# pepborrell/cool-chic

Hardware: AMD Instinct MI355X
Metric: decoded Mpixel/s (Synth+ARM+upsample) @1280x720, all GPUs (higher is better)
Workload: dtype f32; 1 GPU; 1280x720 YUV420 8-bit frames, hop/c3x decoder (arm 16x2, syn 48-1/3-1/3-3r/3-3r, 7 latent grids), float forward ARM+rate -> upsampling -> synthesis -> 420 post; parallelism=image-parallel x1, kernels=ARM | upsampling pyramid | fused last-upsampling+synthesis+post (one stream)

## Files before the change

cool-chic_amd/csrc/fwd_syn.hip:

```cpp
#include <stdlib.h>
#include <type_traits>

#include "fwd_common.h"

using namespace ccmi_fwd;

namespace {

constexpr int kThreads = 256;


#ifndef CCMI_FUSED_RH
#define CCMI_FUSED_RH 32
#endif
#ifndef CCMI_FUSED_THREADS
#define CCMI_FUSED_THREADS 512
#endif
constexpr int kFThreads = CCMI_FUSED_THREADS;
constexpr int kRW = 64, kRH = CCMI_FUSED_RH;
constexpr int kRowsPerThread = kRH / (kFThreads / kRW);
constexpr int kNW = kFThreads / 64;

__device__ __forceinline__ float *at(float *base, uint32_t i) { return (float *)((char *)base + i * 4u); }
__device__ __forceinline__ float ldu(const float *base, uint64_t byte) { return *(const float *)((const char *)base + byte); }
__device__ __forceinline__ uint64_t off64(uint32_t byte, uint32_t z)
{
    uint64_t o = ((uint64_t)z << 32) | byte;
    asm volatile("" : "+v"(o));
    return o;
}

__device__ __forceinline__ void store_out(const FusedArgs &A, float *out, int64_t plane, int m, int gy, int gx, float v,
                                          const float *lut8)
{
    const uint32_t pl = (uint32_t)plane, px = (uint32_t)(gy * A.W + gx);
    if (A.qmax <= 0.f) {
        *at(out, m * pl + px) = v;
        return;
    }
    const float q = lut8 ? lut8[(int)fminf(fmaxf(rintf(v * 255.f), 0.f), 255.f)]
                         : fminf(fmaxf(rintf(v * A.qmax) / A.qmax, 0.f), 1.f);
    if (!A.yuv420 || m == 0) {
        *at(out, m * pl + px) = q;
    } else if (!(gy & 1) && !(gx & 1) && (gy >> 1) < (A.H >> 1) && (gx >> 1) < (A.W >> 1)) {
        const uint32_t cp = (uint32_t)((A.H >> 1) * (A.W >> 1));
        *at(out, pl + (m - 1) * cp + (uint32_t)((gy >> 1) * (A.W >> 1) + (gx >> 1))) = q;
    }
}

typedef float v4f __attribute__((ext_vector_type(4)));
__device__ __forceinline__ v4f mfma16(float a, float b, v4f c) { return __builtin_amdgcn_mfma_f32_16x16x4f32(a, b, c, 0, 0, 0); }

__device__ __forceinline__ void rows_transpose4(const float (&v)[4], float (&t)[4])
{
    const auto p = __builtin_amdgcn_permlane16_swap(__float_as_uint(v[0]), __float_as_uint(v[1]), false, false);
    const auto q = __builtin_amdgcn_permlane16_swap(__float_as_uint(v[2]), __float_as_uint(v[3]), false, false);
    const auto a = __builtin_amdgcn_permlane32_swap(p[0], q[0], false, false);
    const auto b = __builtin_amdgcn_permlane32_swap(p[1], q[1], false, false);
    t[0] = __uint_as_float(a[0]);
    t[1] = __uint_as_float(b[0]);
    t[2] = __uint_as_float(a[1]);
    t[3] = __uint_as_float(b[1]);
}

typedef const __attribute__((address_space(4))) char *kernarg_ptr;
__device__ __forceinline__ kernarg_ptr fresh_kernargs()
{
    kernarg_ptr p = (kernarg_ptr)__builtin_amdgcn_kernarg_segment_ptr();
    asm volatile("" : "+s"(p));
    return p;
}

#if defined(CCMI_ARM_STAMPS)
__device__ unsigned long long g_fstamp[8];
#define FSTAMP(k)                                                                  \
    do {                                                                           \
        __syncthreads();                                                           \
        const unsigned long long _t = __builtin_amdgcn_s_memtime();                \
        if (threadIdx.x == 0) atomicAdd(&g_fstamp[k], _t - t_prev);                \
        t_prev = _t;                                                               \
    } while (0)
#else
#define FSTAMP(k)
#endif

using FT = UpsTile<8, 7, kRH, kRW>;
constexpr int kHsRows = kRH / 2 + 1 + FT::NS - 1;
constexpr int kHrRows = kRH + 7 - 1;
constexpr int kSW = kRW / 2 + 1 + FT::NS - 1 + 3;
constexpr int kTW = kRW + 7 - 1 + 2;

constexpr int fused_groups(int cin, bool ups) { return ups && cin - 1 >= 4 ? 2 : 1; }
constexpr int fused_carry_floats(int cmid) { return kMaxSp * 2 * cmid * kRW; }
constexpr int fused_lds_floats(int cin, int cmid, bool ups)
{
    const int C = ups ? cin - 1 : 0, GC = (C + fused_groups(cin, ups) - 1) / fused_groups(cin, ups);
    const int raw = ups ? GC * kHsRows * kSW + kHrRows * kTW : 0;
    const int stage = ups ? GC * kHsRows * kRW + kHrRows * kRW : 0;
    const int xr = 2 * cmid * kFThreads;
    const int b0 = xr > raw ? xr : raw;
    int b1 = xr > stage ? xr : stage;
    b1 = b1 > kMaxHid * 16 + 256 ? b1 : kMaxHid * 16 + 256;
    return b0 + b1 + fused_carry_floats(cmid) + 256;
}
constexpr int fused_wpe(int cin, int cmid, bool ups, bool mh = false)
{
#ifdef CCMI_FUSED_WPE
    if (!mh) return CCMI_FUSED_WPE;
#endif
    return !mh && 4 * fused_lds_floats(cin, cmid, ups) <= 160 * 1024 / 3 ? 6 : 4;
}

template <int CIN, int CMID, bool UPS, bool MH = false, int HID = 0, bool FOLD = false>
__global__ __launch_bounds__(kFThreads) __attribute__((amdgpu_waves_per_eu(fused_wpe(CIN, CMID, UPS, MH)))) void syn_fused_kernel(FusedArgs Ak, LevelArgs Uk, LevelArgs U2k)
{
    static_assert(!FOLD || (UPS && CIN >= 3), "the fold needs the fused level-1 -> 0 step and a level-2 stack");
    constexpr int NR = kRowsPerThread;
    constexpr int C = UPS ? CIN - 1 : 0, NG = fused_groups(CIN, UPS), GC = (C + NG - 1) / NG;
    constexpr int kRaw = UPS ? GC * kHsRows * kSW + kHrRows * kTW : 0;
    constexpr int kBuf0 = 2 * CMID * kFThreads > kRaw ? 2 * CMID * kFThreads : kRaw;
    constexpr int kTot = fused_lds_floats(CIN, CMID, UPS);
    __shared__ __attribute__((aligned(16))) float s_pool[kTot];
    float *s_st = s_pool;
    float *s_yt = s_st + GC * kHsRows * kSW;
    float *s_hs = s_pool + kBuf0;
    float *s_hr = s_hs + GC * kHsRows * kRW;
    float *s_lut8 = s_pool + kTot - 256;
    float *s_carry = s_lut8 - fused_carry_floats(CMID);
#if defined(CCMI_ARM_STAMPS)
    unsigned long long t_prev = __builtin_amdgcn_s_memtime();
#endif
    float(*s_head)[16] = reinterpret_cast<float(*)[16]>(s_pool + kBuf0);
    float *s_w1p = s_pool + kBuf0 + kMaxHid * 16;
    static_assert(CIN + 1 + CMID <= 16, "hidden-unit record");
    constexpr int kRecVecs = (CIN + 1 + CMID + 3) / 4;

    const int wt = xcd_order(blockIdx.x, gridDim.x);
    const int b0 = wt / Ak.ntiles, tile = wt - b0 * Ak.ntiles;
    const int ri = tile / Ak.tiles_x;
    const int nwin = Ak.run_base + (ri < Ak.run_extra ? 1 : 0);
    const int y0 = kRH * (ri * Ak.run_base + min(ri, Ak.run_extra)) - 2 * Ak.n_sp * ri;
    const int x0 = (tile - ri * Ak.tiles_x) * (kRW - 2 * Ak.n_sp);
    const int oy0 = y0 - Ak.n_sp, ox0 = x0 - Ak.n_sp;
    if (Ak.qmax == 255.f) s_lut8[threadIdx.x & 255] = (float)(threadIdx.x & 255) / 255.f;
#pragma clang loop unroll(disable)
    for (int win = 0; win < nwin; ++win) {
    auto tixf = []() __attribute__((always_inline)) {
        int t = threadIdx.x;
        asm volatile("" : "+v"(t));
        return t;
    };
    const auto kargs = fresh_kernargs();
    constexpr size_t kOffU = (sizeof(FusedArgs) + alignof(LevelArgs) - 1) / alignof(LevelArgs) * alignof(LevelArgs);
    constexpr size_t kOffU2 = (kOffU + sizeof(LevelArgs) + alignof(LevelArgs) - 1) / alignof(LevelArgs) * alignof(LevelArgs);
    const FusedArgs &A = *(const FusedArgs *)kargs;
    const LevelArgs &U = *(const LevelArgs *)(kargs + kOffU);
    const LevelArgs &U2 = *(const LevelArgs *)(kargs + kOffU2);
    const int halo = A.n_sp;
    int b = b0, ox = ox0;
    asm volatile("" : "+s"(b), "+s"(ox));
    const int oy = oy0 + kRH * win;
    const cfloat_ptr prm = (cfloat_ptr)(size_t)(A.params + (int64_t)b * A.pstride);
    const float *in = A.in + (int64_t)b * A.in_stride;
    float *out = A.out + (int64_t)b * A.out_stride;
    const int64_t plane = (int64_t)A.H * A.W;
    int c, rb, gx, cxg;
    auto reidx = [&]() {
        int t = threadIdx.x;
        asm volatile("" : "+v"(t));
        c = t & (kRW - 1);
        rb = (t >> 6) * NR;
        gx = ox + c;
        cxg = clampi(gx, A.W - 1);
    };

    const float *lut8 = A.qmax == 255.f ? s_lut8 : nullptr;
    constexpr int kHeadRegs = (kMaxHid * 16 + kFThreads - 1) / kFThreads;
    constexpr bool kScaledRelu = HID > 0 && !MH;
    constexpr float kW0Scale = kScaledRelu ? 0x1p-32f : 1.f, kW1Scale = kScaledRelu ? 0x1p32f : 1.f;
    float hv[kHeadRegs];
    auto load_head = [&]() {
        const int tid = tixf();
#pragma unroll
        for (int k = 0; k < kHeadRegs; ++k) {
            const int i = tid + k * kFThreads, j = i >> 4, f = i & 15;
            float v = 0.f;
            if (i < kMaxHid * 16 && A.n_head == 2 && j < A.hid) {
                if (f < CIN) v = prm[A.w0_off + j * CIN + f] * kW0Scale;
                else if (f == CIN) v = prm[A.b0_off + j] * kW0Scale;
                else if (f <= CIN + CMID) v = prm[A.w1_off + (f - CIN - 1) * A.hid + j] * kW1Scale;
            }
            hv[k] = v;
        }
    };
    auto stage_head = [&]() {
        const int tid = tixf();
#pragma unroll
        for (int k = 0; k < kHeadRegs; ++k) {
            const int i = tid + k * kFThreads, j = i >> 4, f = i & 15;
            if (i < kMaxHid * 16 && f <= CIN + CMID) s_head[j][f] = hv[k];
        }
        if constexpr (MH) {
            constexpr int n = (HID / 16) * 4 * CMID * 4;
            static_assert(n <= kFThreads, "one entry per thread");
            const int i = tid;
            if (i < n) {
                const int u4 = i & 3, m = (i >> 2) % CMID, lgi = (i / (4 * CMID)) & 3, mt = i / (16 * CMID);
                s_w1p[i] = prm[A.w1_off + m * A.hid + 16 * mt + 4 * lgi + u4];
            }
        }
    };
    reidx();
    if constexpr (!UPS) {
        load_head();
        stage_head();
        __syncthreads();
    }

    float x[NR][CIN];
    const int Ya = clampi(oy, A.H - 1), Xa = clampi(ox, A.W - 1);
    const bool interior = oy >= 0 && oy + kRH <= A.H;
    if constexpr (UPS) {
        float wu[8], wr[7];
        const cfloat_ptr uprm = (cfloat_ptr)(size_t)(U.params + (int64_t)b * U.pstride);
#pragma unroll
        for (int k = 0; k < 8; ++k) wu[k] = uprm[U.up_off + k];
#pragma unroll
        for (int k = 0; k < 7; ++k) wr[k] = uprm[U.pre_off + k];
        const int jbase = Ya / 2 + FT::D0, ibase = Xa / 2 + FT::D0;
        const int wv = __builtin_amdgcn_readfirstlane((int)(tixf() >> 6));
        const int lane = tixf() & 63;
        constexpr int kSR = GC * kHsRows, kSU = (kSR + kNW - 1) / kNW;
        constexpr int kLU = (kHrRows + kNW - 1) / kNW;
        static_assert(kSW <= 64 && kTW <= 128 && kTW > 64 && kHsRows >= kNW, "lane = raw column, one row wrap per step");
        const float *src = U.src + (int64_t)b * U.src_stride;
        const float *rs = U.ref_src + (int64_t)b * U.ref_stride;
        float sv[NG][kSU], tv[kLU][2];
        bool tin[2];
        {
            const int splane = U.hs * U.ws;
            const uint32_t zhi = (uint32_t)tixf() >> 31;
            const uint64_t scol = off64(4u * (uint32_t)clampi(ibase + (lane < kSW ? lane : kSW - 1), U.ws - 1), zhi);
#pragma unroll
            for (int G = 0; G < NG; ++G)
#pragma unroll
                for (int u = 0; u < kSU; ++u) {
                    if constexpr (FOLD) break;
                    const int r = wv + kNW * u;
                    const int c0 = (kNW * u) / kHsRows, tb = kHsRows * (c0 + 1) - kNW * u;
                    const int lc = c0 + (wv >= tb ? 1 : 0), jj = r - lc * kHsRows;
                    sv[G][u] = 0.f;
                    if ((u < kSU - 1 || r < kSR) && G * GC + lc < C) {
                        const int row = (G * GC + lc) * splane + clampi(jbase + jj, U.hs - 1) * U.ws;
#if defined(CCMI_DIAG_NOLOAD)
                        sv[G][u] = 0.001f * (float)(jj + scol);
#else
                        sv[G][u] = ldu(src + row, scol);
#endif
                    }
                }
            uint64_t tx[2];
#pragma unroll
            for (int h = 0; h < 2; ++h) {
                const int X = Xa - 3 + (lane + 64 * h < kTW ? lane + 64 * h : kTW - 1);
                tin[h] = X >= 0 && X < U.wd;
                tx[h] = off64(4u * (uint32_t)clampi(X, U.wd - 1), zhi);
            }
#pragma unroll
            for (int u = 0; u < kLU; ++u) {
                const int yr = wv + kNW * u;
                const int Y = Ya - 3 + yr;
                const int row = clampi(Y, U.hd - 1) * U.wd;
#pragma unroll
                for (int h = 0; h < 2; ++h) {
#if defined(CCMI_DIAG_NOLOAD)
                    tv[u][h] = 0.001f * (float)(yr + tx[h]);
#else
                    tv[u][h] = ldu(rs + row, tx[h]);
#endif
                }
            }
        }
        if constexpr (FOLD) {
            constexpr int C2 = CIN - 2;
            constexpr int kFLR = kHsRows + 6, kFLW = kSW + 6, kFLP = kFLW + 1;
            constexpr int kFP = 40;
            constexpr int kF2R = (kHsRows - 1) / 2 + 1 + FT::NS - 1;
            constexpr int kF2W = (kSW - 1) / 2 + 1 + FT::NS - 1, kF2P = kF2W + 1;
            static_assert(kFP >= kSW, "pass pitch");
            float *f_lat = s_pool;
            float *f_ref = f_lat + kFLR * kFLP;
            float *f_src = f_ref + kFLR * kFP;
            float *f_h2 = f_src + C2 * kF2R * kF2P;
            static_assert(kFLR * kFLP + kFLR * kFP + C2 * kF2R * (kF2P + kFP) <= kTot - 256 - fused_carry_floats(CMID), "fold tiles fit before the carry rows");
            const int hs1 = U.hs, ws1 = U.ws, hs2 = U2.hs, ws2 = U2.ws;
            const int R0 = clampi(jbase, hs1 - 1), R1 = clampi(jbase + kHsRows - 1, hs1 - 1);
            const int C0 = clampi(ibase, ws1 - 1);
            const int r2 = (R0 >> 1) + FT::D0, c2 = (C0 >> 1) + FT::D0;
            const cfloat_ptr uprm2 = (cfloat_ptr)(size_t)(U2.params + (int64_t)b * U2.pstride);
            float wu2[8], wr2[7];
#pragma unroll
            for (int k = 0; k < 8; ++k) wu2[k] = uprm2[U2.up_off + k];
#pragma unroll
            for (int k = 0; k < 7; ++k) wr2[k] = uprm2[U2.pre_off + k];
            const int tid = tixf();
            {
                const float *l1 = U2.ref_src + (int64_t)b * U2.ref_stride;
                const float *s2 = U2.src + (int64_t)b * U2.src_stride;
                constexpr int NL = (kFLR * kFLW + kFThreads - 1) / kFThreads;
                constexpr int NS2 = (C2 * kF2R * kF2W + kFThreads - 1) / kFThreads;
                float lv[NL], sv2[NS2];
#pragma unroll
                for (int u = 0; u < NL; ++u) {
                    const int i = tid + u * kFThreads, r = i / kFLW, c = i - r * kFLW;
                    const int Y = R0 - 3 + r, X = C0 - 3 + c;
                    lv[u] = (i < kFLR * kFLW && Y >= 0 && Y < hs1 && X >= 0 && X < ws1) ? l1[Y * ws1 + X] : 0.f;
                }
#pragma unroll
                for (int u = 0; u < NS2; ++u) {
                    const int i = tid + u * kFThreads, ch = i / (kF2R * kF2W), rem = i - ch * (kF2R * kF2W);
                    const int r = rem / kF2W, c = rem - r * kF2W;
                    sv2[u] = i < C2 * kF2R * kF2W
                                 ? s2[(ch * hs2 + clampi(r2 + r, hs2 - 1)) * ws2 + clampi(c2 + c, ws2 - 1)]
                                 : 0.f;
                }
#pragma unroll
                for (int u = 0; u < NL; ++u) {
                    const int i = tid + u * kFThreads, r = i / kFLW, c = i - r * kFLW;
                    if (i < kFLR * kFLW) f_lat[r * kFLP + c] = U2.ref_quant ? rintf(U2.gain * lv[u]) : lv[u];
                }
#pragma unroll
                for (int u = 0; u < NS2; ++u) {
                    const int i = tid + u * kFThreads, ch = i / (kF2R * kF2W), rem = i - ch * (kF2R * kF2W);
                    const int r = rem / kF2W, c = rem - r * kF2W;
                    if (i < C2 * kF2R * kF2W) f_src[(ch * kF2R + r) * kF2P + c] = U2.src_quant ? rintf(U2.gain * sv2[u]) : sv2[u];
                }
            }
            __syncthreads();
            for (int i = tid; i < kFLR * kSW; i += kFThreads) {
                const int r = i / kSW, c = i - r * kSW;
                const float *p = f_lat + r * kFLP + c;
                float acc = 0.f;
#pragma unroll
                for (int k = 0; k < 7; ++k) acc = fmaf(wr2[k], p[k], acc);
                f_ref[r * kFP + c] = acc;
            }
            {
                constexpr int NQ = kSW / 2 + 1;
                const int q0 = C0 >> 1;
                for (int i = tid; i < C2 * kF2R * NQ; i += kFThreads) {
                    const int ch = i / (kF2R * NQ), rem = i - ch * (kF2R * NQ), r = rem / NQ, q = rem - r * NQ;
                    const float *p = f_src + (ch * kF2R + r) * kF2P + q;
                    float e = 0.f, o = 0.f;
#pragma unroll
                    for (int m = 0; m < FT::NS; ++m) {
// ... 63 lines not shown
            constexpr int G = decltype(GI)::value;
            if constexpr (G > 0) __syncthreads();
#pragma unroll
            for (int u = 0; u < kSU; ++u) {
                const int r = wv + kNW * u;
                if ((u < kSU - 1 || r < kSR) && lane < kSW)
                    s_st[r * kSW + lane] = U.src_quant ? rintf(U.gain * sv[G][u]) : sv[G][u];
            }
            if constexpr (G == 0) {
#pragma unroll
                for (int u = 0; u < kLU; ++u) {
                    const int yr = wv + kNW * u;
                    if (yr >= kHrRows) continue;
                    const int Y = Ya - 3 + yr;
                    const bool yin = Y >= 0 && Y < U.hd;
#pragma unroll
                    for (int h = 0; h < 2; ++h) {
                        const float v = U.ref_quant ? rintf(U.gain * tv[u][h]) : tv[u][h];
                        if (lane + 64 * h < kTW) s_yt[yr * kTW + lane + 64 * h] = (yin && tin[h]) ? v : 0.f;
                    }
                }
            }
            __builtin_amdgcn_fence(__ATOMIC_RELEASE, "wavefront");
            __builtin_amdgcn_wave_barrier();
            __builtin_amdgcn_fence(__ATOMIC_ACQUIRE, "wavefront");
            if constexpr (G == 0) FSTAMP(0);
            {
                const int odd = Xa & 1;
                const int k = lane & 31, hsel = lane >> 5;
                const int xe = 2 * k - odd;
                static_assert(32 + FT::NS - 1 < kSW, "pair 32 reads stay inside the source row");
                auto pair = [&](int r, int kk, int xw) {
                    const float *sr = s_st + r * kSW + kk;
                    f2 eo = f2(0.f);
#pragma unroll
                    for (int m = 0; m < FT::NS; ++m) eo = __builtin_elementwise_fma(wp[m], f2(sr[m]), eo);
                    float *hrow = s_hs + r * kRW;
                    if (xw >= 0) hrow[xw] = eo.x;
                    if (xw + 1 < kRW) hrow[xw + 1] = eo.y;
                };
#pragma unroll
                for (int u = 0; u < kSU; u += 2) {
                    const int r = wv + kNW * (u + hsel);
                    if (u + 1 < kSU - 1 || r < kSR) pair(r, k, xe);
                }
                if (odd) {
                    const int r = wv + kNW * lane;
                    if (lane < kSU && r < kSR) pair(r, 32, 63);
                }
                if constexpr (G == 0) {
#pragma unroll
                    for (int u = 0; u < kLU; ++u) {
                        const int yr = wv + kNW * u;
                        if (yr >= kHrRows) continue;
                        const float *tr = s_yt + yr * kTW + lane;
                        float acc = 0.f;
#pragma unroll
                        for (int q = 0; q < 7; ++q) acc = fmaf(wr[q], tr[q], acc);
                        s_hr[yr * kRW + lane] = acc;
                    }
                }
            }
            __syncthreads();
            if constexpr (G == 0) FSTAMP(1);
            const int xi = cxg - Xa;
            if (interior) {
                auto gather = [&](auto par) {
                    constexpr int P = decltype(par)::value;
                    if constexpr (G == 0) {
                        float h[NR + 6];
#pragma unroll
                        for (int k = 0; k < NR + 6; ++k) h[k] = s_hr[(rb + k) * kRW + xi];
#pragma unroll
                        for (int p = 0; p < NR; ++p) {
                            float acc = 0.f;
#pragma unroll
                            for (int k = 0; k < 7; ++k) acc = fmaf(wr[k], h[p + k], acc);
                            x[p][0] = acc + s_yt[(rb + p + 3) * kTW + xi + 3];
                        }
                    }
                    constexpr int NH = FT::NS + (NR / 2) - 1 + P;
                    const int j0 = rb / 2;
#pragma unroll
                    for (int lc = 0; lc < GC; ++lc) {
                        constexpr int dummy = 0;
                        (void)dummy;
                        const int k = 1 + G * GC + lc;
                        if (k >= CIN) break;
                        float h[NH];
#pragma unroll
                        for (int m = 0; m < NH; ++m) h[m] = s_hs[(lc * kHsRows + j0 + m) * kRW + xi];
#pragma unroll
                        for (int p = 0; p < NR; ++p) {
                            const int a = (P + p) & 1, off = (P + p) >> 1;
                            float acc = 0.f;
#pragma unroll
                            for (int m = 0; m < FT::NS; ++m) {
                                const int te = FT::tap(0, FT::D0 + m), to = FT::tap(1, FT::D0 + m);
                                if ((a ? to : te) >= 0) acc = fmaf(wu[a ? to : te], h[off + m], acc);
                            }
                            x[p][k] = acc;
                        }
                    }
                };
                if (oy & 1) gather(std::integral_constant<int, 1>{});
                else gather(std::integral_constant<int, 0>{});
            } else {
#pragma unroll
                for (int p = 0; p < NR; ++p) {
                    const int Y = clampi(oy + rb + p, A.H - 1);
                    const int yi = Y - Ya;
                    if constexpr (G == 0) {
                        float acc = 0.f;
#pragma unroll
                        for (int k = 0; k < 7; ++k) acc = fmaf(wr[k], s_hr[(yi + k) * kRW + xi], acc);
                        x[p][0] = acc + s_yt[(yi + 3) * kTW + xi + 3];
                    }
                    const int jj0 = Y / 2 - Ya / 2, a = Y & 1;
#pragma unroll
                    for (int lc = 0; lc < GC; ++lc) {
                        const int k = 1 + G * GC + lc;
                        if (k >= CIN) break;
                        const float *h = s_hs + (lc * kHsRows + jj0) * kRW + xi;
                        float acc_e = 0.f, acc_o = 0.f;
#pragma unroll
                        for (int m = 0; m < FT::NS; ++m) {
                            const int te = FT::tap(0, FT::D0 + m), to = FT::tap(1, FT::D0 + m);
                            const float hv = h[m * kRW];
                            if (te >= 0) acc_e = fmaf(wu[te], hv, acc_e);
                            if (to >= 0) acc_o = fmaf(wu[to], hv, acc_o);
                        }
                        x[p][k] = a ? acc_o : acc_e;
                    }
                }
            }
        };
        if constexpr (NG > 1) {
            group(std::integral_constant<int, 0>{});
            load_head();
            group(std::integral_constant<int, 1>{});
        } else {
            load_head();
            group(std::integral_constant<int, 0>{});
        }
    } else {
#pragma unroll
        for (int p = 0; p < NR; ++p) {
            const int64_t pix = (int64_t)clampi(oy + rb + p, A.H - 1) * A.W + cxg;
#pragma unroll
            for (int k = 0; k < CIN; ++k) x[p][k] = in[k * plane + pix];
        }
    }

    f2 img[NR / 2][CMID];
    {
        const FusedArgs &A = *(const FusedArgs *)fresh_kernargs();
        const cfloat_ptr w0 = prm + A.w0_off, b0 = prm + A.b0_off;
        const cfloat_ptr b1 = prm + A.b1_off;
        float o[NR][CMID];
        if constexpr (UPS) {
            __syncthreads();
            stage_head();
        }
        FSTAMP(2);
        if constexpr (MH) {
            static_assert(HID % 16 == 0 && HID <= kMaxHid && CIN + 1 <= 8 && CMID <= 4, "f32-MFMA head shape");
            constexpr int NT = HID / 16;
            const int lane = tixf() & 63, lr = lane & 15, lg = lane >> 4;
            __syncthreads();
            float a1[NT][2];
#pragma unroll
            for (int mt = 0; mt < NT; ++mt)
#pragma unroll
                for (int k = 0; k < 2; ++k) {
                    const int ch = 4 * k + lg;
                    a1[mt][k] = ch <= CIN ? s_head[16 * mt + lr][ch] : 0.f;
                }
            const f2 lo0 = f2(A.relu0 ? 0.f : -INFINITY);
            const float lo1 = A.relu1 ? 0.f : -INFINITY;
            typedef const __attribute__((address_space(3))) v4f *lds_v4;
            lds_v4 wb = (lds_v4)s_w1p;
            asm volatile("" : "+v"(wb));
#pragma unroll
            for (int p = 0; p < NR; ++p) {
                asm volatile("" : "+v"(wb));
                float T[2][4];
                {
                    float v0[4], v1[4];
#pragma unroll
                    for (int k = 0; k < 4; ++k) {
                        v0[k] = k < CIN ? x[p][k] : (k == CIN ? 1.f : 0.f);
                        v1[k] = 4 + k < CIN ? x[p][4 + k] : (4 + k == CIN ? 1.f : 0.f);
                    }
                    rows_transpose4(v0, T[0]);
                    rows_transpose4(v1, T[1]);
                }
                float P[4][CMID];
#pragma unroll
                for (int gh = 0; gh < 2; ++gh) {
                    f2 P2[2][CMID];
#pragma unroll
                    for (int gi = 0; gi < 2; ++gi)
#pragma unroll
                        for (int m = 0; m < CMID; ++m) P2[gi][m] = f2(0.f);
#pragma unroll
                    for (int mt = 0; mt < NT; ++mt) {
                        v4f w[CMID];
#pragma unroll
                        for (int m = 0; m < CMID; ++m) w[m] = wb[(mt * 4 + lg) * CMID + m];
#pragma unroll
                        for (int gi = 0; gi < 2; ++gi) {
                            const int g = 2 * gh + gi;
                            v4f acc = mfma16(a1[mt][0], T[0][g], v4f{0.f, 0.f, 0.f, 0.f});
                            acc = mfma16(a1[mt][1], T[1][g], acc);
                            const f2 h01 = __builtin_elementwise_max(f2{acc[0], acc[1]}, lo0);
                            const f2 h23 = __builtin_elementwise_max(f2{acc[2], acc[3]}, lo0);
#pragma unroll
                            for (int m = 0; m < CMID; ++m) {
                                P2[gi][m] = __builtin_elementwise_fma(f2{w[m][0], w[m][1]}, h01, P2[gi][m]);
                                P2[gi][m] = __builtin_elementwise_fma(f2{w[m][2], w[m][3]}, h23, P2[gi][m]);
                            }
                        }
                    }
#pragma unroll
                    for (int gi = 0; gi < 2; ++gi)
#pragma unroll
                        for (int m = 0; m < CMID; ++m) P[2 * gh + gi][m] = P2[gi][m].x + P2[gi][m].y;
                }
#pragma unroll
                for (int m = 0; m < CMID; ++m) {
                    const float v[4] = {P[0][m], P[1][m], P[2][m], P[3][m]};
                    float t[4];
                    rows_transpose4(v, t);
                    o[p][m] = fmaxf(((t[0] + t[1]) + (t[2] + t[3])) + b1[m], lo1);
                }
            }
        } else if (A.n_head == 2) {
            const int hid = HID > 0 ? HID : A.hid;
            f2 xp[NR / 2][CIN], op[NR / 2][CMID];
#pragma unroll
            for (int q = 0; q < NR / 2; ++q) {
#pragma unroll
                for (int k = 0; k < CIN; ++k) xp[q][k] = f2{x[2 * q][k], x[2 * q + 1][k]};
#pragma unroll
                for (int m = 0; m < CMID; ++m) op[q][m] = f2(0.f);
            }
            __syncthreads();
            struct Rec { f4v v[kRecVecs]; };
            typedef const __attribute__((address_space(3))) f4v *lds_f4;
            lds_f4 hb = (lds_f4)(&s_head[0][0]);
            asm volatile("" : "+v"(hb));
            auto load = [&](int j) {
                const lds_f4 p = hb + 4 * (j < hid ? j : hid - 1);
                Rec r;
#pragma unroll
                for (int i = 0; i < kRecVecs; ++i) r.v[i] = p[i];
                return r;
            };
            const f2 lo0 = f2(A.relu0 ? 0.f : -INFINITY);
            constexpr bool RELU = kScaledRelu;
            constexpr int NQ = NR / 2;
            static_assert(NQ % 2 == 0, "the head's statements take two pixel pairs");
            auto hidden = [&](const Rec &r, f2(&h)[NQ]) __attribute__((always_inline)) {
                f2 w[4];
                rec_w0_pairs<CIN>(r.v, w);
#pragma unroll
                for (int q = 0; q < NQ; q += 2) {
                    head_hidden2<CIN, RELU>(w, rec_pair<CIN>(r.v), xp[q], xp[q + 1], h[q], h[q + 1]);
                    if constexpr (!RELU) {
                        h[q] = __builtin_elementwise_max(h[q], lo0);
                        h[q + 1] = __builtin_elementwise_max(h[q + 1], lo0);
                    }
                }
            };
            auto outs = [&](const Rec &r, const f2(&h)[NQ]) __attribute__((always_inline)) {
                static_for<CMID>([&](auto mc) __attribute__((always_inline)) {
                    constexpr int m = decltype(mc)::value, S = CIN + 1 + m;
#pragma unroll
                    for (int q = 0; q < NQ; q += 2) head_out2<S & 1>(rec_pair<S>(r.v), h[q], h[q + 1], op[q][m], op[q + 1][m]);
                });
            };
            if constexpr (HID > 0) {
                constexpr int kHidVecs = CIN / 4 + 1;
                auto read = [&](Rec &r, int j, int v0, int v1) __attribute__((always_inline)) {
#pragma unroll
                    for (int i = v0; i < v1; ++i) r.v[i] = hb[4 * j + i];
                };
                Rec cur, nxt;
                read(cur, 0, 0, kRecVecs);
                nxt = cur;
#pragma unroll
                for (int j = 0; j < HID; ++j) {
                    f2 h[NQ];
                    if (j + 1 < HID) read(nxt, j + 1, 0, kHidVecs);
                    hidden(cur, h);
                    if (j + 1 < HID) read(nxt, j + 1, kHidVecs, kRecVecs);
                    outs(cur, h);
                    cur = nxt;
                }
            } else {
                auto unit = [&](const Rec &r) __attribute__((always_inline)) {
                    f2 h[NQ];
                    hidden(r, h);
                    outs(r, h);
                };
                Rec ra = load(0), rb2 = load(1);
                for (int j = 0; j < hid; j += 2) {
                    unit(ra);
                    ra = load(j + 2);
                    if (j + 1 < hid) unit(rb2);
                    rb2 = load(j + 3);
                }
            }
            const float lo1 = A.relu1 ? 0.f : -INFINITY;
#pragma unroll
            for (int q = 0; q < NR / 2; ++q)
#pragma unroll
                for (int m = 0; m < CMID; ++m) {
                    o[2 * q][m] = fmaxf(op[q][m].x + b1[m], lo1);
                    o[2 * q + 1][m] = fmaxf(op[q][m].y + b1[m], lo1);
                }
        } else {
            const float lo0 = A.relu0 ? 0.f : -INFINITY;
#pragma unroll
            for (int m = 0; m < CMID; ++m) {
                const float bm = b0[m];
#pragma unroll
                for (int p = 0; p < NR; ++p) {
                    float acc = bm;
#pragma unroll
                    for (int k = 0; k < CIN; ++k) acc = fmaf(w0[m * CIN + k], x[p][k], acc);
                    o[p][m] = fmaxf(acc, lo0);
                }
            }
        }
        FSTAMP(3);
        reidx();
        if (halo == 0) {
#pragma unroll
            for (int p = 0; p < NR; ++p) {
                const int gy = oy + rb + p;
                if (gy < A.H && gx < A.W)
#pragma unroll
                    for (int m = 0; m < CMID; ++m) store_out(A, out, plane, m, gy, gx, o[p][m], lut8);
            }
        }
#pragma unroll
        for (int q = 0; q < NR / 2; ++q)
#pragma unroll
            for (int m = 0; m < CMID; ++m) img[q][m] = f2{o[2 * q][m], o[2 * q + 1][m]};
    }

    if (halo != 0) {
    const FusedArgs &A = *(const FusedArgs *)fresh_kernargs();
    float *xb0 = s_pool, *xb1 = s_pool + kBuf0;
    auto publish = [&](float *xb) __attribute__((always_inline)) {
        const int tid = tixf();
#pragma unroll
        for (int m = 0; m < CMID; ++m) {
            xb[m * kFThreads + tid] = img[NR / 2 - 1][m].x;
            xb[(CMID + m) * kFThreads + tid] = img[NR / 2 - 1][m].y;
        }
    };
    auto shr1 = [](float v) __attribute__((always_inline)) {
        return __int_as_float(__builtin_amdgcn_update_dpp(0, __float_as_int(v), 0x138, 0xf, 0xf, true));
    };
    auto shl1 = [](float v) __attribute__((always_inline)) {
        return __int_as_float(__builtin_amdgcn_update_dpp(0, __float_as_int(v), 0x130, 0xf, 0xf, true));
    };
    const bool rows_inner = oy - halo - 1 >= 0 && oy + kRH <= A.H;
    const bool cols_inner = ox >= 0 && ox + kRW <= A.W;
    auto layer = [&](auto LAST, int s, const float *xin, float *xout) __attribute__((always_inline)) {
        constexpr bool last = decltype(LAST)::value;
        const int tid = tixf();
        const int wrow = __builtin_amdgcn_readfirstlane(tid >> 6) * NR;
        float *cr = s_carry + s * (2 * CMID * kRW) + (tid & (kRW - 1));
        float v[NR + 2][CMID];
        if (wrow == 0) {
#pragma unroll
            for (int m = 0; m < CMID; ++m) {
                v[0][m] = cr[m * kRW];
                v[1][m] = cr[(CMID + m) * kRW];
            }
        }
        __syncthreads();
        const cfloat_ptr wt = prm + A.sp[s].w_off;
        const cfloat_ptr bs = prm + A.sp[s].b_off;
        const f2 lo = f2(A.sp[s].relu ? 0.f : -INFINITY);
        const f2 rsd = f2(A.sp[s].residual ? 1.f : 0.f);
        if (wrow != 0) {
#pragma unroll
            for (int m = 0; m < CMID; ++m) {
                v[0][m] = xin[m * kFThreads + tid - kRW];
                v[1][m] = xin[(CMID + m) * kFThreads + tid - kRW];
            }
        }
#pragma unroll
        for (int m = 0; m < CMID; ++m)
#pragma unroll
            for (int p = 0; p < NR; ++p) v[p + 2][m] = (p & 1) ? img[p / 2][m].y : img[p / 2][m].x;
        if (wrow == kRH - NR) {
#pragma unroll
            for (int m = 0; m < CMID; ++m) {
                cr[m * kRW] = v[NR][m];
                cr[(CMID + m) * kRW] = v[NR + 1][m];
            }
        }
        if (!rows_inner) {
            const int gy0 = oy + wrow - 2 - s;
#pragma unroll
            for (int i = 1; i < NR + 2; ++i)
                if (gy0 + i >= A.H)
#pragma unroll
                    for (int m = 0; m < CMID; ++m) v[i][m] = v[i - 1][m];
#pragma unroll
            for (int i = NR; i >= 0; --i)
                if (gy0 + i < 0)
#pragma unroll
                    for (int m = 0; m < CMID; ++m) v[i][m] = v[i + 1][m];
        }
        f2 P[NR + 1][CMID];
#pragma unroll
        for (int r = 0; r <= NR; ++r)
#pragma unroll
            for (int k = 0; k < CMID; ++k) P[r][k] = f2{v[r][k], v[r + 1][k]};
        f2 nxt[NR / 2][CMID];
#pragma unroll
        for (int m = 0; m < CMID; ++m) {
            const cfloat_ptr wm = wt + m * CMID * 9;
            f2 S[3][NR / 2];
#pragma unroll
            for (int q = 0; q < NR / 2; ++q) {
                S[0][q] = f2(0.f);
                S[1][q] = f2(bs[m]);
                S[2][q] = f2(0.f);
            }
#pragma unroll
            for (int k = 0; k < CMID; ++k)
#pragma unroll
                for (int dy = 0; dy < 3; ++dy)
#pragma unroll
                    for (int dx = 0; dx < 3; ++dx) {
                        const f2 w = f2(wm[(k * 3 + dy) * 3 + dx]);
#pragma unroll
                        for (int q = 0; q < NR / 2; ++q) S[dx][q] = __builtin_elementwise_fma(w, P[2 * q + dy][k], S[dx][q]);
                    }
#pragma unroll
            for (int q = 0; q < NR / 2; ++q) {
                f2 acc;
                acc.x = (S[1][q].x + shr1(S[0][q].x)) + shl1(S[2][q].x);
                acc.y = (S[1][q].y + shr1(S[0][q].y)) + shl1(S[2][q].y);
                nxt[q][m] = __builtin_elementwise_max(__builtin_elementwise_fma(rsd, P[2 * q + 1][m], acc), lo);
            }
        }
#pragma unroll
        for (int q = 0; q < NR / 2; ++q)
#pragma unroll
            for (int m = 0; m < CMID; ++m) img[q][m] = nxt[q][m];
        if constexpr (!last) {
            if (!cols_inner) {
                const int c0 = -ox, c1 = A.W - 1 - ox;
                const int lane = tid & 63;
#pragma unroll
                for (int q = 0; q < NR / 2; ++q)
#pragma unroll
                    for (int m = 0; m < CMID; ++m) {
                        float e0 = img[q][m].x, e1 = img[q][m].y;
                        if (c0 > 0) {
                            const float l0 = __int_as_float(__builtin_amdgcn_readlane(__float_as_int(e0), c0));
                            const float l1 = __int_as_float(__builtin_amdgcn_readlane(__float_as_int(e1), c0));
                            e0 = lane < c0 ? l0 : e0;
                            e1 = lane < c0 ? l1 : e1;
                        }
                        if (c1 < kRW - 1) {
                            const float r0 = __int_as_float(__builtin_amdgcn_readlane(__float_as_int(e0), c1));
                            const float r1 = __int_as_float(__builtin_amdgcn_readlane(__float_as_int(e1), c1));
                            e0 = lane > c1 ? r0 : e0;
                            e1 = lane > c1 ? r1 : e1;
                        }
                        img[q][m] = f2{e0, e1};
                    }
            }
            publish(xout);
        }
    };
    publish(xb0);
    for (int s = 0; s < A.n_sp - 1; ++s) {
        layer(std::false_type{}, s, xb0, xb1);
        float *const t = xb0;
        xb0 = xb1;
        xb1 = t;
    }
    layer(std::true_type{}, A.n_sp - 1, xb0, nullptr);
    {
        reidx();
        const int t = A.n_sp;
        const bool col_ok = c >= t && c < kRW - t && gx < A.W;
        const uint32_t pl = (uint32_t)plane;
        const uint32_t cw = (uint32_t)(A.W >> 1), cp = (uint32_t)((A.H >> 1) * (A.W >> 1));
        const bool cx_ok = !(gx & 1) && (gx >> 1) < (A.W >> 1);
        auto emit = [&](auto MODE) {
            constexpr int md = decltype(MODE)::value;
            constexpr bool tab = md >= 3;
            constexpr int fmt = tab ? md - 2 : md;
#pragma unroll
            for (int p = 0; p < NR; ++p) {
                const int r = rb + p, gy = oy + r - t;
                if (!(col_ok && (win > 0 || r >= 2 * t) && gy < A.H)) continue;
                const uint32_t px = (uint32_t)(gy * A.W + gx);
                const bool cy_ok = fmt == 2 && cx_ok && !(gy & 1) && (gy >> 1) < (A.H >> 1);
                const uint32_t cpx = (uint32_t)((gy >> 1) * (int)cw + (gx >> 1));
#pragma unroll
                for (int m = 0; m < CMID; ++m) {
                    if (fmt == 2 && m > 0 && (gy & 1)) break;
                    float v = (p & 1) ? img[p / 2][m].y : img[p / 2][m].x;
                    if constexpr (fmt > 0) {
                        v = tab ? lut8[(int)fminf(fmaxf(rintf(v * 255.f), 0.f), 255.f)]
                                : fminf(fmaxf(rintf(v * A.qmax) / A.qmax, 0.f), 1.f);
                    }
                    if (fmt < 2 || m == 0) *at(out, m * pl + px) = v;
                    else if (cy_ok) *at(out, pl + (m - 1) * cp + cpx) = v;
                }
            }
        };
        if (A.qmax <= 0.f) emit(std::integral_constant<int, 0>{});
        else if (lut8) {
            if (A.yuv420) emit(std::integral_constant<int, 4>{});
            else emit(std::integral_constant<int, 3>{});
        } else if (A.yuv420) emit(std::integral_constant<int, 2>{});
        else emit(std::integral_constant<int, 1>{});
    }
    }
    FSTAMP(4);
    __syncthreads();
    }
}

__global__ __launch_bounds__(kThreads) void syn_layer_kernel(const float *__restrict__ in, int64_t in_stride, int cin,
                                                             int H, int W, const float *__restrict__ params,
                                                             int64_t pstride, int w_off, int b_off, int nout, int ks,
                                                             int residual, int relu, float *__restrict__ out,
                                                             int64_t out_stride)
{
    const int b = blockIdx.y;
    const int64_t plane = (int64_t)H * W;
    const int64_t p = (int64_t)blockIdx.x * kThreads + threadIdx.x;
    if (p >= plane) return;
    const int y = (int)(p / W), x = (int)(p - (int64_t)y * W);
    const float *src = in + (int64_t)b * in_stride;
    float *dst = out + (int64_t)b * out_stride;
    const float *wt = params + (int64_t)b * pstride + w_off;
    const float *bs = params + (int64_t)b * pstride + b_off;
    const int pad = ks / 2;
    for (int m = 0; m < nout; ++m) {
        float acc = 0.f;
        for (int k = 0; k < cin; ++k)
            for (int dy = 0; dy < ks; ++dy) {
                const int yy = clampi(y + dy - pad, H - 1);
                for (int dx = 0; dx < ks; ++dx) {
                    const int xx = clampi(x + dx - pad, W - 1);
                    acc = fmaf(wt[((m * cin + k) * ks + dy) * ks + dx], src[k * plane + (int64_t)yy * W + xx], acc);
                }
            }
        float v = acc + bs[m];
        if (residual) v += src[m * plane + p];
        if (relu) v = fmaxf(v, 0.f);
        dst[m * plane + p] = v;
    }
}

__global__ __launch_bounds__(kThreads) void post_kernel(const float *__restrict__ in, int64_t in_stride, int H, int W,
                                                        float qmax, int yuv420, float *__restrict__ out,
                                                        int64_t out_stride)
{
    const int b = blockIdx.y;
    const int64_t plane = (int64_t)H * W;
    const int64_t p = (int64_t)blockIdx.x * kThreads + threadIdx.x;
    if (p >= plane) return;
    const float *src = in + (int64_t)b * in_stride;
    float *dst = out + (int64_t)b * out_stride;
    auto q = [qmax](float v) { return fminf(fmaxf(rintf(v * qmax) / qmax, 0.f), 1.f); };
    dst[p] = q(src[p]);
    const int y = (int)(p / W), x = (int)(p - (int64_t)y * W);
    if (!yuv420) {
        dst[plane + p] = q(src[plane + p]);
        dst[2 * plane + p] = q(src[2 * plane + p]);
    } else if (!(y & 1) && !(x & 1) && y / 2 < H / 2 && x / 2 < W / 2) {
        const int64_t cp = (int64_t)(H / 2) * (W / 2);
        const int64_t ci = (int64_t)(y / 2) * (W / 2) + x / 2;
        dst[plane + ci] = q(src[plane + p]);
        dst[plane + cp + ci] = q(src[2 * plane + p]);
    }
}

bool unrolled_head(const FusedArgs &fa) { return fa.cin == 7 && fa.n_head == 2 && fa.hid == 48 && fa.relu0 && !fa.head_generic; }

template <int CMID, bool UPS>
void launch_fused(dim3 grid, hipStream_t s, const FusedArgs &fa, const LevelArgs &u)
{
    const LevelArgs none{};
    if (unrolled_head(fa)) {
        hipLaunchKernelGGL((syn_fused_kernel<7, CMID, UPS, false, 48>), grid, dim3(kFThreads), 0, s, fa, u, none);
        return;
    }
    switch (fa.cin) {
    case 1: hipLaunchKernelGGL((syn_fused_kernel<1, CMID, false>), grid, dim3(kFThreads), 0, s, fa, u, none); break;
#define CCMI_FUSED_CASE(N) \
    case N: hipLaunchKernelGGL((syn_fused_kernel<N, CMID, UPS>), grid, dim3(kFThreads), 0, s, fa, u, none); break;
    CCMI_FUSED_CASE(2) CCMI_FUSED_CASE(3) CCMI_FUSED_CASE(4) CCMI_FUSED_CASE(5) CCMI_FUSED_CASE(6)
    CCMI_FUSED_CASE(7) CCMI_FUSED_CASE(8)
#undef CCMI_FUSED_CASE
    }
}

template <int CMID>
bool launch_fused_mfma_head(dim3 grid, hipStream_t s, const FusedArgs &fa, const LevelArgs &u)
{
    if (!fa.head_mfma || fa.cin != 7 || fa.n_head != 2 || fa.hid != 48 || fa.n_sp < 1) return false;
    hipLaunchKernelGGL((syn_fused_kernel<7, CMID, true, true, 48>), grid, dim3(kFThreads), 0, s, fa, u, LevelArgs{});
    return true;
}

bool fold_eligible(const FusedArgs &fa, int cmid) { return cmid == 3 && unrolled_head(fa) && !fa.head_mfma; }

void set_runs(FusedArgs &f, int cap)
{
    const RunPlan rp = fused_run_plan(f.H, f.n_sp, cap, kRH);
    f.tiles_x = ccmi_div_up(f.W, kRW - 2 * f.n_sp);
    f.ntiles = f.tiles_x * rp.n_runs;
    f.run_base = rp.base;
    f.run_extra = rp.extra;
}

}

namespace ccmi_fwd {

void layer_offsets(const ccmi_syn_args *a, int *w_off, int *b_off, int *cin_of, int64_t *total)
{
    int64_t o = 0;
    int c = a->c_in;
    for (int l = 0; l < a->n_layers; ++l) {
        const ccmi_syn_layer &L = a->layers[l];
        cin_of[l] = c;
        w_off[l] = (int)o;
        o += (int64_t)L.n_out * c * L.ks * L.ks;
        b_off[l] = (int)o;
        o += L.n_out;
        c = L.n_out;
    }
    *total = o;
}

bool make_plan(const ccmi_syn_args *a, Plan *P)
{
    int w_off[CCMI_MAX_SYN_LAYERS], b_off[CCMI_MAX_SYN_LAYERS], cin_of[CCMI_MAX_SYN_LAYERS];
    int64_t tot;
    layer_offsets(a, w_off, b_off, cin_of, &tot);
    P->fused = false;
    const ccmi_syn_layer *L = a->layers;
    int n_head = 0;
    while (n_head < a->n_layers && n_head < 2 && L[n_head].ks == 1 && !L[n_head].residual) n_head++;
    if (n_head == 0 || a->c_in > kMaxIn) return false;
    const int cmid = L[n_head - 1].n_out;
    if (cmid < 1 || cmid > kMaxMid) return false;
    int hid = n_head == 2 ? L[0].n_out : 0;
    if (hid > kMaxHid) return false;
    const int n_sp = a->n_layers - n_head;
// ... 188 lines not shown
```

Measured before the change: 27710 Mpixel/s.

## Skip odd-row chroma in last synthesis layer for YUV420 and repack rows

```diff
diff --git a/cool-chic_amd/csrc/fwd_syn.hip b/cool-chic_amd/csrc/fwd_syn.hip
--- a/cool-chic_amd/csrc/fwd_syn.hip
+++ b/cool-chic_amd/csrc/fwd_syn.hip
@@ -87,15 +87,16 @@
 using FT = UpsTile<8, 7, kRH, kRW>;
 constexpr int kHsRows = kRH / 2 + 1 + FT::NS - 1;
 constexpr int kHrRows = kRH + 7 - 1;
-constexpr int kSW = kRW / 2 + 1 + FT::NS - 1 + 3;
+constexpr int kSW = kRW / 2 + 1 + FT::NS - 1 + 2;
 constexpr int kTW = kRW + 7 - 1 + 2;
 
 constexpr int fused_groups(int cin, bool ups) { return ups && cin - 1 >= 4 ? 2 : 1; }
 constexpr int fused_carry_floats(int cmid) { return kMaxSp * 2 * cmid * kRW; }
+constexpr int fused_raw_floats(int gc) { return (gc * kHsRows * kSW + kHrRows * kTW + 3) / 4 * 4; }
 constexpr int fused_lds_floats(int cin, int cmid, bool ups)
 {
     const int C = ups ? cin - 1 : 0, GC = (C + fused_groups(cin, ups) - 1) / fused_groups(cin, ups);
-    const int raw = ups ? GC * kHsRows * kSW + kHrRows * kTW : 0;
+    const int raw = ups ? fused_raw_floats(GC) : 0;
     const int stage = ups ? GC * kHsRows * kRW + kHrRows * kRW : 0;
     const int xr = 2 * cmid * kFThreads;
     const int b0 = xr > raw ? xr : raw;
@@ -110,6 +111,15 @@
 #endif
     return !mh && 4 * fused_lds_floats(cin, cmid, ups) <= 160 * 1024 / 3 ? 6 : 4;
 }
+#ifndef CCMI_FUSED_RUN_RECS
+#define CCMI_FUSED_RUN_RECS 0
+#endif
+constexpr int kRunRecPitch = 12;
+constexpr bool fused_run_recs(int cin, int cmid, bool ups, bool mh, int hid)
+{
+    return CCMI_FUSED_RUN_RECS && ups && !mh && hid > 0 && fused_groups(cin, ups) == 2 && cin + 1 + cmid <= kRunRecPitch &&
+           4 * (fused_lds_floats(cin, cmid, ups) + kRunRecPitch * hid) <= 160 * 1024 / 3;
+}
 
 template <int CIN, int CMID, bool UPS, bool MH = false, int HID = 0, bool FOLD = false>
 __global__ __launch_bounds__(kFThreads) __attribute__((amdgpu_waves_per_eu(fused_wpe(CIN, CMID, UPS, MH)))) void syn_fused_kernel(FusedArgs Ak, LevelArgs Uk, LevelArgs U2k)
@@ -117,10 +127,13 @@
     static_assert(!FOLD || (UPS && CIN >= 3), "the fold needs the fused level-1 -> 0 step and a level-2 stack");
     constexpr int NR = kRowsPerThread;
     constexpr int C = UPS ? CIN - 1 : 0, NG = fused_groups(CIN, UPS), GC = (C + NG - 1) / NG;
-    constexpr int kRaw = UPS ? GC * kHsRows * kSW + kHrRows * kTW : 0;
+    constexpr int kRaw = UPS ? fused_raw_floats(GC) : 0;
     constexpr int kBuf0 = 2 * CMID * kFThreads > kRaw ? 2 * CMID * kFThreads : kRaw;
     constexpr int kTot = fused_lds_floats(CIN, CMID, UPS);
-    __shared__ __attribute__((aligned(16))) float s_pool[kTot];
+    constexpr bool kRunRecs = fused_run_recs(CIN, CMID, UPS, MH, HID);
+    constexpr int kRecPitch = kRunRecs ? kRunRecPitch : 16;
+    static_assert(kBuf0 % 4 == 0 && kTot % 4 == 0, "the records are read as 128-bit words");
+    __shared__ __attribute__((aligned(16))) float s_pool[kTot + (kRunRecs ? kRunRecPitch * HID : 0)];
     float *s_st = s_pool;
     float *s_yt = s_st + GC * kHsRows * kSW;
     float *s_hs = s_pool + kBuf0;
@@ -130,9 +143,9 @@
 #if defined(CCMI_ARM_STAMPS)
     unsigned long long t_prev = __builtin_amdgcn_s_memtime();
 #endif
-    float(*s_head)[16] = reinterpret_cast<float(*)[16]>(s_pool + kBuf0);
+    float *s_head = s_pool + (kRunRecs ? kTot : kBuf0);
     float *s_w1p = s_pool + kBuf0 + kMaxHid * 16;
-    static_assert(CIN + 1 + CMID <= 16, "hidden-unit record");
+    static_assert(CIN + 1 + CMID <= kRecPitch, "hidden-unit record");
     constexpr int kRecVecs = (CIN + 1 + CMID + 3) / 4;
 
     const int wt = xcd_order(blockIdx.x, gridDim.x);
@@ -143,13 +156,45 @@
     const int x0 = (tile - ri * Ak.tiles_x) * (kRW - 2 * Ak.n_sp);
     const int oy0 = y0 - Ak.n_sp, ox0 = x0 - Ak.n_sp;
     if (Ak.qmax == 255.f) s_lut8[threadIdx.x & 255] = (float)(threadIdx.x & 255) / 255.f;
-#pragma clang loop unroll(disable)
-    for (int win = 0; win < nwin; ++win) {
     auto tixf = []() __attribute__((always_inline)) {
         int t = threadIdx.x;
         asm volatile("" : "+v"(t));
         return t;
     };
+    constexpr int kHeadRegs = (kMaxHid * 16 + kFThreads - 1) / kFThreads;
+    constexpr bool kScaledRelu = HID > 0 && !MH;
+    constexpr float kW0Scale = kScaledRelu ? 0x1p-32f : 1.f, kW1Scale = kScaledRelu ? 0x1p32f : 1.f;
+    auto fetch_recs = [&](const FusedArgs &A, cfloat_ptr prm, float(&hv)[kHeadRegs]) __attribute__((always_inline)) {
+        const int tid = tixf();
+#pragma unroll
+        for (int k = 0; k < kHeadRegs; ++k) {
+            const int i = tid + k * kFThreads, j = i >> 4, f = i & 15;
+            float v = 0.f;
+            if (i < kMaxHid * 16 && A.n_head == 2 && j < A.hid) {
+                if (f < CIN) v = prm[A.w0_off + j * CIN + f] * kW0Scale;
+                else if (f == CIN) v = prm[A.b0_off + j] * kW0Scale;
+                else if (f <= CIN + CMID) v = prm[A.w1_off + (f - CIN - 1) * A.hid + j] * kW1Scale;
+            }
+            hv[k] = v;
+        }
+    };
+    auto store_recs = [&](const float(&hv)[kHeadRegs]) __attribute__((always_inline)) {
+        const int tid = tixf();
+        constexpr int kUnits = kRunRecs ? HID : kMaxHid;
+#pragma unroll
+        for (int k = 0; k < kHeadRegs; ++k) {
+            const int i = tid + k * kFThreads, j = i >> 4, f = i & 15;
+            if (j < kUnits && f <= CIN + CMID) s_head[j * kRecPitch + f] = hv[k];
+        }
+    };
+    if constexpr (kRunRecs) {
+        const FusedArgs &A = *(const FusedArgs *)fresh_kernargs();
+        float hv[kHeadRegs];
+        fetch_recs(A, (cfloat_ptr)(size_t)(A.params + (int64_t)b0 * A.pstride), hv);
+        store_recs(hv);
+    }
+#pragma clang loop unroll(disable)
+    for (int win = 0; win < nwin; ++win) {
     const auto kargs = fresh_kernargs();
     constexpr size_t kOffU = (sizeof(FusedArgs) + alignof(LevelArgs) - 1) / alignof(LevelArgs) * alignof(LevelArgs);
     constexpr size_t kOffU2 = (kOffU + sizeof(LevelArgs) + alignof(LevelArgs) - 1) / alignof(LevelArgs) * alignof(LevelArgs);
@@ -175,32 +220,14 @@
     };
 
     const float *lut8 = A.qmax == 255.f ? s_lut8 : nullptr;
-    constexpr int kHeadRegs = (kMaxHid * 16 + kFThreads - 1) / kFThreads;
-    constexpr bool kScaledRelu = HID > 0 && !MH;
-    constexpr float kW0Scale = kScaledRelu ? 0x1p-32f : 1.f, kW1Scale = kScaledRelu ? 0x1p32f : 1.f;
     float hv[kHeadRegs];
     auto load_head = [&]() {
-        const int tid = tixf();
-#pragma unroll
-        for (int k = 0; k < kHeadRegs; ++k) {
-            const int i = tid + k * kFThreads, j = i >> 4, f = i & 15;
-            float v = 0.f;
-            if (i < kMaxHid * 16 && A.n_head == 2 && j < A.hid) {
-                if (f < CIN) v = prm[A.w0_off + j * CIN + f] * kW0Scale;
-                else if (f == CIN) v = prm[A.b0_off + j] * kW0Scale;
-                else if (f <= CIN + CMID) v = prm[A.w1_off + (f - CIN - 1) * A.hid + j] * kW1Scale;
-            }
-            hv[k] = v;
-        }
+        if constexpr (!kRunRecs) fetch_recs(A, prm, hv);
     };
     auto stage_head = [&]() {
-        const int tid = tixf();
-#pragma unroll
-        for (int k = 0; k < kHeadRegs; ++k) {
-            const int i = tid + k * kFThreads, j = i >> 4, f = i & 15;
-            if (i < kMaxHid * 16 && f <= CIN + CMID) s_head[j][f] = hv[k];
-        }
+        if constexpr (!kRunRecs) store_recs(hv);
         if constexpr (MH) {
+            const int tid = tixf();
             constexpr int n = (HID / 16) * 4 * CMID * 4;
             static_assert(n <= kFThreads, "one entry per thread");
             const int i = tid;
@@ -570,13 +597,16 @@
         }
     }
 
-    f2 img[NR / 2][CMID];
+    constexpr int NP = NR / 2;
+    static_assert(NR % 4 == 0, "a pair's rows have one parity");
+    f2 img[NP][CMID];
+    auto row_of = [&](int p, int m) __attribute__((always_inline)) { return p < NP ? img[p][m].x : img[p - NP][m].y; };
     {
         const FusedArgs &A = *(const FusedArgs *)fresh_kernargs();
         const cfloat_ptr w0 = prm + A.w0_off, b0 = prm + A.b0_off;
         const cfloat_ptr b1 = prm + A.b1_off;
         float o[NR][CMID];
-        if constexpr (UPS) {
+        if constexpr (UPS && !kRunRecs) {
             __syncthreads();
             stage_head();
         }
@@ -592,7 +622,7 @@
 #pragma unroll
                 for (int k = 0; k < 2; ++k) {
                     const int ch = 4 * k + lg;
-                    a1[mt][k] = ch <= CIN ? s_head[16 * mt + lr][ch] : 0.f;
+                    a1[mt][k] = ch <= CIN ? s_head[(16 * mt + lr) * kRecPitch + ch] : 0.f;
                 }
             const f2 lo0 = f2(A.relu0 ? 0.f : -INFINITY);
             const float lo1 = A.relu1 ? 0.f : -INFINITY;
@@ -659,17 +689,18 @@
 #pragma unroll
             for (int q = 0; q < NR / 2; ++q) {
 #pragma unroll
-                for (int k = 0; k < CIN; ++k) xp[q][k] = f2{x[2 * q][k], x[2 * q + 1][k]};
+                for (int k = 0; k < CIN; ++k) xp[q][k] = f2{x[q][k], x[q + NR / 2][k]};
 #pragma unroll
                 for (int m = 0; m < CMID; ++m) op[q][m] = f2(0.f);
             }
-            __syncthreads();
+            if constexpr (!kRunRecs) __syncthreads();
             struct Rec { f4v v[kRecVecs]; };
             typedef const __attribute__((address_space(3))) f4v *lds_f4;
-            lds_f4 hb = (lds_f4)(&s_head[0][0]);
+            constexpr int kRecStep = kRecPitch / 4;
+            lds_f4 hb = (lds_f4)s_head;
             asm volatile("" : "+v"(hb));
             auto load = [&](int j) {
-                const lds_f4 p = hb + 4 * (j < hid ? j : hid - 1);
+                const lds_f4 p = hb + kRecStep * (j < hid ? j : hid - 1);
                 Rec r;
 #pragma unroll
                 for (int i = 0; i < kRecVecs; ++i) r.v[i] = p[i];
@@ -702,7 +733,7 @@
                 constexpr int kHidVecs = CIN / 4 + 1;
                 auto read = [&](Rec &r, int j, int v0, int v1) __attribute__((always_inline)) {
 #pragma unroll
-                    for (int i = v0; i < v1; ++i) r.v[i] = hb[4 * j + i];
+                    for (int i = v0; i < v1; ++i) r.v[i] = hb[kRecStep * j + i];
                 };
                 Rec cur, nxt;
                 read(cur, 0, 0, kRecVecs);
@@ -735,8 +766,8 @@
             for (int q = 0; q < NR / 2; ++q)
 #pragma unroll
                 for (int m = 0; m < CMID; ++m) {
-                    o[2 * q][m] = fmaxf(op[q][m].x + b1[m], lo1);
-                    o[2 * q + 1][m] = fmaxf(op[q][m].y + b1[m], lo1);
+                    o[q][m] = fmaxf(op[q][m].x + b1[m], lo1);
+                    o[q + NR / 2][m] = fmaxf(op[q][m].y + b1[m], lo1);
                 }
         } else {
             const float lo0 = A.relu0 ? 0.f : -INFINITY;
@@ -766,7 +797,7 @@
 #pragma unroll
         for (int q = 0; q < NR / 2; ++q)
 #pragma unroll
-            for (int m = 0; m < CMID; ++m) img[q][m] = f2{o[2 * q][m], o[2 * q + 1][m]};
+            for (int m = 0; m < CMID; ++m) img[q][m] = f2{o[q][m], o[q + NR / 2][m]};
     }
 
     if (halo != 0) {
@@ -776,8 +807,8 @@
         const int tid = tixf();
 #pragma unroll
         for (int m = 0; m < CMID; ++m) {
-            xb[m * kFThreads + tid] = img[NR / 2 - 1][m].x;
-            xb[(CMID + m) * kFThreads + tid] = img[NR / 2 - 1][m].y;
+            xb[m * kFThreads + tid] = row_of(NR - 2, m);
+            xb[(CMID + m) * kFThreads + tid] = row_of(NR - 1, m);
         }
     };
     auto shr1 = [](float v) __attribute__((always_inline)) {
@@ -788,8 +819,9 @@
     };
     const bool rows_inner = oy - halo - 1 >= 0 && oy + kRH <= A.H;
     const bool cols_inner = ox >= 0 && ox + kRW <= A.W;
-    auto layer = [&](auto LAST, int s, const float *xin, float *xout) __attribute__((always_inline)) {
+    auto layer = [&](auto LAST, bool c420, int s, const float *xin, float *xout) __attribute__((always_inline)) {
         constexpr bool last = decltype(LAST)::value;
+        static_assert(kRH % 2 == 0, "row parity");
         const int tid = tixf();
         const int wrow = __builtin_amdgcn_readfirstlane(tid >> 6) * NR;
         float *cr = s_carry + s * (2 * CMID * kRW) + (tid & (kRW - 1));
@@ -816,7 +848,7 @@
 #pragma unroll
         for (int m = 0; m < CMID; ++m)
 #pragma unroll
-            for (int p = 0; p < NR; ++p) v[p + 2][m] = (p & 1) ? img[p / 2][m].y : img[p / 2][m].x;
+            for (int p = 0; p < NR; ++p) v[p + 2][m] = row_of(p, m);
         if (wrow == kRH - NR) {
 #pragma unroll
             for (int m = 0; m < CMID; ++m) {
@@ -837,18 +869,17 @@
 #pragma unroll
                     for (int m = 0; m < CMID; ++m) v[i][m] = v[i + 1][m];
         }
-        f2 P[NR + 1][CMID];
-#pragma unroll
-        for (int r = 0; r <= NR; ++r)
-#pragma unroll
-            for (int k = 0; k < CMID; ++k) P[r][k] = f2{v[r][k], v[r + 1][k]};
-        f2 nxt[NR / 2][CMID];
-#pragma unroll
-        for (int m = 0; m < CMID; ++m) {
+        f2 E[NP + 2][CMID];
+#pragma unroll
+        for (int i = 0; i < NP + 2; ++i)
+#pragma unroll
+            for (int k = 0; k < CMID; ++k) E[i][k] = f2{v[i][k], v[i + NP][k]};
+        f2 nxt[NP][CMID];
+        auto chan = [&](cfloat_ptr wt, cfloat_ptr bs, int m, int qa, int qs) __attribute__((always_inline)) {
             const cfloat_ptr wm = wt + m * CMID * 9;
-            f2 S[3][NR / 2];
-#pragma unroll
-            for (int q = 0; q < NR / 2; ++q) {
+            f2 S[3][NP];
+#pragma unroll
+            for (int q = qa; q < NP; q += qs) {
                 S[0][q] = f2(0.f);
                 S[1][q] = f2(bs[m]);
                 S[2][q] = f2(0.f);
@@ -861,15 +892,37 @@
                     for (int dx = 0; dx < 3; ++dx) {
                         const f2 w = f2(wm[(k * 3 + dy) * 3 + dx]);
 #pragma unroll
-                        for (int q = 0; q < NR / 2; ++q) S[dx][q] = __builtin_elementwise_fma(w, P[2 * q + dy][k], S[dx][q]);
-                    }
-#pragma unroll
-            for (int q = 0; q < NR / 2; ++q) {
+                        for (int q = qa; q < NP; q += qs) S[dx][q] = __builtin_elementwise_fma(w, E[q + dy][k], S[dx][q]);
+                    }
+#pragma unroll
+            for (int q = qa; q < NP; q += qs) {
                 f2 acc;
                 acc.x = (S[1][q].x + shr1(S[0][q].x)) + shl1(S[2][q].x);
                 acc.y = (S[1][q].y + shr1(S[0][q].y)) + shl1(S[2][q].y);
-                nxt[q][m] = __builtin_elementwise_max(__builtin_elementwise_fma(rsd, P[2 * q + 1][m], acc), lo);
-            }
+                nxt[q][m] = __builtin_elementwise_max(__builtin_elementwise_fma(rsd, E[q + 1][m], acc), lo);
+            }
+        };
+        if constexpr (last && CMID == 3) {
+            chan(wt, bs, 0, 0, 1);
+#pragma unroll
+            for (int m = 1; m < CMID; ++m) {
+                chan(wt, bs, m, 0, 2);
+#pragma unroll
+                for (int q = 1; q < NP; q += 2) nxt[q][m] = f2(0.f);
+            }
+#pragma unroll
+            for (int m = 0; m < CMID; ++m)
+#pragma unroll
+                for (int q = 0; q < NP; q += (m > 0 ? 2 : 1)) asm volatile("" : "+v"(nxt[q][m]));
+            if (!c420) {
+                cfloat_ptr wt2 = wt, bs2 = bs;
+                asm volatile("" : "+s"(wt2), "+s"(bs2));
+#pragma unroll
+                for (int m = 1; m < CMID; ++m) chan(wt2, bs2, m, 1, 2);
+            }
+        } else {
+#pragma unroll
+            for (int m = 0; m < CMID; ++m) chan(wt, bs, m, 0, 1);
         }
 #pragma unroll
         for (int q = 0; q < NR / 2; ++q)
@@ -904,12 +957,12 @@
     };
     publish(xb0);
     for (int s = 0; s < A.n_sp - 1; ++s) {
-        layer(std::false_type{}, s, xb0, xb1);
+        layer(std::false_type{}, false, s, xb0, xb1);
         float *const t = xb0;
         xb0 = xb1;
         xb1 = t;
     }
-    layer(std::true_type{}, A.n_sp - 1, xb0, nullptr);
+    layer(std::true_type{}, A.yuv420 && A.qmax > 0.f, A.n_sp - 1, xb0, nullptr);
     {
         reidx();
         const int t = A.n_sp;
@@ -930,8 +983,8 @@
                 const uint32_t cpx = (uint32_t)((gy >> 1) * (int)cw + (gx >> 1));
 #pragma unroll
                 for (int m = 0; m < CMID; ++m) {
-                    if (fmt == 2 && m > 0 && (gy & 1)) break;
-                    float v = (p & 1) ? img[p / 2][m].y : img[p / 2][m].x;
+                    if (fmt == 2 && m > 0 && (p & 1)) break;
+                    float v = row_of(p, m);
                     if constexpr (fmt > 0) {
                         v = tab ? lut8[(int)fminf(fmaxf(rintf(v * 255.f), 0.f), 255.f)]
                                 : fminf(fmaxf(rintf(v * A.qmax) / A.qmax, 0.f), 1.f);
```

New measurement: 28180 Mpixel/s (median of 6 runs). 1.7% higher.
